# hydradarpa/kalman-hydra

Hardware: AMD Instinct MI355X
Metric: frames/sec (Brox flow + EKF update) at 1024^2 (higher is better)
Workload: dtype f32 (flow, renders) / f64 (EKF sums and state)

## Files before the change

include/hydra_mi.h:

```cpp
#ifndef HYDRA_MI_H
#define HYDRA_MI_H

#include <stdint.h>

#ifdef __cplusplus
extern "C" {
#endif

#define HM_OK 0
#define HM_ERR_ARG (-1)
#define HM_ERR_HIP (-2)
#define HM_ERR_STATE (-3)
#define HM_ERR_NUMERIC (-4)

const char *hm_last_error(void);
const char *hm_version(void);
int hm_device_count(void);

int hm_dev_alloc(int device, uint64_t bytes, void **out);
int hm_dev_free(int device, void *ptr);
int hm_dev_upload(int device, void *dst, const void *src, uint64_t bytes);
int hm_dev_download(int device, void *dst, const void *src, uint64_t bytes);
int hm_copy_stream_create(int device, void **stream_out);
int hm_copy_stream_destroy(int device, void *stream);
// ... 75 lines not shown
int hm_update_step(hm_ctx_t h, const double *X, double deltaX, int masked, double *step, double *Hzc,
                   double err[4]);
int hm_update_cov(hm_ctx_t h, int which, double *W_out);
int hm_update_run(hm_ctx_t h, const double *W_prior, double *X, double deltaX, int masked, int max_iter,
                  double reltol, int info[4], double *errs, double *Hzc, double *gains, double *W_out);
int hm_cov_fetch(hm_ctx_t h, double *W_out);
int hm_ms_newton(int n_vertices, int n_bars, const int32_t *bars, const double *l0, double kappa, double M,
                 double dt, int maxiter, double tol, double *X, int *newton_iterations);
int hm_ms_worker_create(void **worker);
int hm_ms_worker_destroy(void *worker);
int hm_ms_newton_start(void *worker, int n_vertices, int n_bars, const int32_t *bars, const double *l0, double kappa,
                       double M, double dt, int maxiter, double tol, const double *X);
int hm_ms_newton_finish(void *worker, double *X, int *newton_iterations);
int hm_ms_worker_attach(void *worker, hm_ctx_t ctx);
int hm_newton_dev_start(hm_ctx_t h, int N, int n_bars, const int32_t *bars, const double *l0, double kappa, double M,
                        double dt, int maxiter, double tol, const double *X);
int hm_newton_dev_finish(hm_ctx_t h, double *X, int *newton_iterations);
int hm_update_arm_newton(hm_ctx_t h, void *worker, int n_bars, const int32_t *bars, const double *l0, double kappa,
                         double M, double dt, int maxiter, double tol);
int hm_update_arm_cov(hm_ctx_t h, double eps_F);
int hm_predict_take(hm_ctx_t h, const double *X, int n_bars, const int32_t *bars, const double *l0, double kappa,
                    double a, double s, double eps_F);
int hm_cov_predict(hm_ctx_t h, const double *W_in, int n_bars, const int32_t *bars, const double *blocks,
                   double a, double s, double eps_F, double *W_out);
int hm_ms_predict(hm_ctx_t h, int n_bars, const int32_t *bars, const double *l0, double kappa, double M, double dt,
                  int maxiter, double tol, double eps_F, double *X, int *newton_iterations, int prefactor);
int hm_update_last_error(hm_ctx_t h, const double *X, double err[4]);
int hm_chain_project(hm_ctx_t h);
int hm_prepare_mask(hm_ctx_t h, const uint8_t *d_y_m);
int hm_update_arm_mask(hm_ctx_t h, const uint8_t *d_y_m);
int hm_update_tail(hm_ctx_t h, double *Hzc, double *gains);
int hm_chain_states(hm_ctx_t h, double *predicted, double *projected, int *newton_iterations, int *moved);
int hm_ctx_tune(hm_ctx_t h, const char *key, int value);
int hm_ctx_sync(hm_ctx_t h);
void *hm_ctx_stream(hm_ctx_t h);

typedef struct hm_smooth *hm_smooth_t;
int hm_smooth_create(hm_ctx_t ctx, int capacity, int n_bars, const int32_t *bars, const double *l0, double kappa,
                     double a, double s, double eps_F, hm_smooth_t *out);
int hm_smooth_destroy(hm_smooth_t sm);
int hm_smooth_record(hm_smooth_t sm, const double *X);
int hm_smooth_run(hm_smooth_t sm, int want_cov, double *xs, double *var);
int hm_smooth_count(hm_smooth_t sm, int *frames, int *capacity);
int hm_smooth_fetch(hm_smooth_t sm, int k, double *P_out, double *x_out, double *m_out);
int hm_smooth_prior(hm_smooth_t sm, int k, double *Pp_out);
int hm_op_smooth_gemm(int device, int which, int n, const double *A, const double *B, const double *C, double *out);

int hm_view(hm_ctx_t h, const double *X, int which, const int32_t *palette, uint8_t *bgr);
int hm_view_dev(hm_ctx_t h, const double *X, int which, const int32_t *palette, void *d_bgr, void *stream);
int hm_view_forces(hm_ctx_t h, const double *X, const double *orig, const double *pred, const double *tv,
                   const double *fv, const double *mv, uint8_t *bgr);

int hm_view_set_cells(hm_ctx_t h, int n_layers, const int32_t *labels, const uint16_t *weights, int L, const uint8_t *colours);
int hm_view_cells(hm_ctx_t h, const double *X, const uint8_t *frame, const uint8_t *levels, int flags,
                  int P, const double *points, const uint8_t *point_colours, int point_radius, uint8_t *bgr);
int hm_view_cells_dev(hm_ctx_t h, const double *X, const void *d_frame, const uint8_t *levels, int flags,
                      int P, const double *points, const uint8_t *point_colours, int point_radius, void *d_bgr, void *stream);

int hm_body_map(hm_ctx_t h, int32_t *tri_of_pixel, uint32_t *tri_counts);
int hm_body_set_labels(hm_ctx_t h, const int32_t *labels, int L, uint32_t *counts);
int hm_body_warp(hm_ctx_t h, const double *X, const uint8_t *frame, uint8_t *out, uint64_t *tri_sums, uint64_t *label_sums);
int hm_body_warp_dev(hm_ctx_t h, const double *X, const void *d_frame, void *d_out, int out_channels,
                     void *d_tri_sums, void *d_label_sums, void *stream);
int hm_body_fence(hm_ctx_t h, void *stream);

int hm_body_stats_begin(hm_ctx_t h);
// ... 42 lines not shown
```

kalman-hydra_amd/_lib.py:

```python
import ctypes
import os

import numpy as np

_HERE = os.path.dirname(os.path.abspath(__file__))
SO_PATH = os.environ.get("HYDRA_MI_SO") or os.path.join(_HERE, "libhydra_mi.so")

c_f32p = ctypes.POINTER(ctypes.c_float)
c_f64p = ctypes.POINTER(ctypes.c_double)
c_u8p = ctypes.POINTER(ctypes.c_uint8)
c_i32p = ctypes.POINTER(ctypes.c_int32)
c_vp = ctypes.c_void_p

SIGNATURES = {
    "hm_last_error": (ctypes.c_char_p, []),
    "hm_version": (ctypes.c_char_p, []),
    "hm_device_count": (ctypes.c_int, []),
    "hm_dev_alloc": (ctypes.c_int, [ctypes.c_int, ctypes.c_uint64, ctypes.POINTER(c_vp)]),
    "hm_dev_free": (ctypes.c_int, [ctypes.c_int, c_vp]),
    "hm_dev_upload": (ctypes.c_int, [ctypes.c_int, c_vp, c_vp, ctypes.c_uint64]),
    "hm_dev_download": (ctypes.c_int, [ctypes.c_int, c_vp, c_vp, ctypes.c_uint64]),
    "hm_copy_stream_create": (ctypes.c_int, [ctypes.c_int, ctypes.POINTER(c_vp)]),
    "hm_copy_stream_destroy": (ctypes.c_int, [ctypes.c_int, c_vp]),
    "hm_copy_stream_sync": (ctypes.c_int, [ctypes.c_int, c_vp]),
# ... 50 lines not shown
    "hm_update_run": (ctypes.c_int, [c_vp, c_vp, c_vp, ctypes.c_double, ctypes.c_int, ctypes.c_int, ctypes.c_double,
                                     ctypes.POINTER(ctypes.c_int), c_vp, c_vp, c_vp, c_vp]),
    "hm_update_last_error": (ctypes.c_int, [c_vp, c_vp, c_f64p]),
    "hm_cov_fetch": (ctypes.c_int, [c_vp, c_vp]),
    "hm_project_mask": (ctypes.c_int, [c_vp, c_vp, c_vp, c_vp]),
    "hm_cov_predict": (ctypes.c_int, [c_vp, c_vp, ctypes.c_int, c_vp, c_vp, ctypes.c_double, ctypes.c_double,
                                      ctypes.c_double, c_vp]),
    "hm_ms_newton": (ctypes.c_int, [ctypes.c_int, ctypes.c_int, c_vp, c_vp, ctypes.c_double, ctypes.c_double,
                                    ctypes.c_double, ctypes.c_int, ctypes.c_double, c_vp, ctypes.POINTER(ctypes.c_int)]),
    "hm_ms_worker_create": (ctypes.c_int, [ctypes.POINTER(c_vp)]),
    "hm_ms_worker_destroy": (ctypes.c_int, [c_vp]),
    "hm_ms_newton_start": (ctypes.c_int, [c_vp, ctypes.c_int, ctypes.c_int, c_vp, c_vp, ctypes.c_double, ctypes.c_double,
                                          ctypes.c_double, ctypes.c_int, ctypes.c_double, c_vp]),
    "hm_ms_newton_finish": (ctypes.c_int, [c_vp, c_vp, ctypes.POINTER(ctypes.c_int)]),
    "hm_ms_worker_attach": (ctypes.c_int, [c_vp, c_vp]),
    "hm_newton_dev_start": (ctypes.c_int, [c_vp, ctypes.c_int, ctypes.c_int, c_vp, c_vp, ctypes.c_double, ctypes.c_double,
                                           ctypes.c_double, ctypes.c_int, ctypes.c_double, c_vp]),
    "hm_newton_dev_finish": (ctypes.c_int, [c_vp, c_vp, ctypes.POINTER(ctypes.c_int)]),
    "hm_prune_mask": (ctypes.c_int, [c_vp, c_vp, c_vp]),
    "hm_chain_project": (ctypes.c_int, [c_vp]),
    "hm_prepare_mask": (ctypes.c_int, [c_vp, c_vp]),
    "hm_update_arm_mask": (ctypes.c_int, [c_vp, c_vp]),
    "hm_update_tail": (ctypes.c_int, [c_vp, c_vp, c_vp]),
    "hm_chain_states": (ctypes.c_int, [c_vp, c_vp, c_vp, ctypes.POINTER(ctypes.c_int), ctypes.POINTER(ctypes.c_int)]),
    "hm_update_arm_newton": (ctypes.c_int, [c_vp, c_vp, ctypes.c_int, c_vp, c_vp, ctypes.c_double, ctypes.c_double,
                                            ctypes.c_double, ctypes.c_int, ctypes.c_double]),
    "hm_update_arm_cov": (ctypes.c_int, [c_vp, ctypes.c_double]),
    "hm_predict_take": (ctypes.c_int, [c_vp, c_vp, ctypes.c_int, c_vp, c_vp, ctypes.c_double, ctypes.c_double,
                                       ctypes.c_double, ctypes.c_double]),
    "hm_ms_predict": (ctypes.c_int, [c_vp, ctypes.c_int, c_vp, c_vp, ctypes.c_double, ctypes.c_double, ctypes.c_double,
                                     ctypes.c_int, ctypes.c_double, ctypes.c_double, c_vp, ctypes.POINTER(ctypes.c_int),
                                     ctypes.c_int]),
    "hm_ctx_tune": (ctypes.c_int, [c_vp, ctypes.c_char_p, ctypes.c_int]),
    "hm_ctx_sync": (ctypes.c_int, [c_vp]),
    "hm_ctx_stream": (c_vp, [c_vp]),
    "hm_smooth_create": (ctypes.c_int, [c_vp, ctypes.c_int, ctypes.c_int, c_vp, c_vp, ctypes.c_double, ctypes.c_double,
                                        ctypes.c_double, ctypes.c_double, ctypes.POINTER(c_vp)]),
    "hm_smooth_destroy": (ctypes.c_int, [c_vp]),
    "hm_smooth_record": (ctypes.c_int, [c_vp, c_vp]),
    "hm_smooth_run": (ctypes.c_int, [c_vp, ctypes.c_int, c_vp, c_vp]),
    "hm_smooth_count": (ctypes.c_int, [c_vp, c_i32p, c_i32p]),
    "hm_smooth_fetch": (ctypes.c_int, [c_vp, ctypes.c_int, c_vp, c_vp, c_vp]),
    "hm_smooth_prior": (ctypes.c_int, [c_vp, ctypes.c_int, c_vp]),
    "hm_op_smooth_gemm": (ctypes.c_int, [ctypes.c_int, ctypes.c_int, ctypes.c_int, c_vp, c_vp, c_vp, c_vp]),
    "hm_view": (ctypes.c_int, [c_vp, c_vp, ctypes.c_int, c_vp, c_vp]),
    "hm_view_dev": (ctypes.c_int, [c_vp, c_vp, ctypes.c_int, c_vp, c_vp, c_vp]),
    "hm_view_forces": (ctypes.c_int, [c_vp, c_vp, c_vp, c_vp, c_vp, c_vp, c_vp, c_vp]),
    "hm_view_set_cells": (ctypes.c_int, [c_vp, ctypes.c_int, c_vp, c_vp, ctypes.c_int, c_vp]),
    "hm_view_cells": (ctypes.c_int, [c_vp, c_vp, c_vp, c_vp, ctypes.c_int, ctypes.c_int, c_vp, c_vp, ctypes.c_int, c_vp]),
    "hm_view_cells_dev": (ctypes.c_int, [c_vp, c_vp, c_vp, c_vp, ctypes.c_int, ctypes.c_int, c_vp, c_vp, ctypes.c_int, c_vp,
                                         c_vp]),
    "hm_body_map": (ctypes.c_int, [c_vp, c_vp, c_vp]),
    "hm_body_set_labels": (ctypes.c_int, [c_vp, c_vp, ctypes.c_int, c_vp]),
    "hm_body_warp": (ctypes.c_int, [c_vp, c_vp, c_vp, c_vp, c_vp, c_vp]),
    "hm_body_warp_dev": (ctypes.c_int, [c_vp, c_vp, c_vp, c_vp, ctypes.c_int, c_vp, c_vp, c_vp]),
    "hm_body_fence": (ctypes.c_int, [c_vp, c_vp]),
    "hm_body_stats_begin": (ctypes.c_int, [c_vp]),
    "hm_body_stats_end": (ctypes.c_int, [c_vp]),
    "hm_body_stats_count": (ctypes.c_int, [c_vp, c_vp]),
    "hm_body_stats_fetch": (ctypes.c_int, [c_vp, c_vp, c_vp, c_vp, c_vp]),
    "hm_body_stats_images": (ctypes.c_int, [c_vp, c_vp, c_vp, c_vp, c_vp]),
    "hm_body_stats_peaks": (ctypes.c_int, [c_vp, ctypes.c_int, ctypes.c_int, ctypes.c_double, ctypes.c_int, c_vp, c_vp,
                                           c_vp]),
    "hm_body_rec_begin": (ctypes.c_int, [c_vp, ctypes.c_uint64]),
    "hm_body_rec_end": (ctypes.c_int, [c_vp]),
    "hm_body_rec_count": (ctypes.c_int, [c_vp, c_vp]),
# ... 121 lines not shown
```

kalman-hydra_amd/csrc/ctx.h:

```cpp
#pragma once
#include "hm_common.h"
#include "hm_types.h"
#include <chrono>
#include <condition_variable>
#include <functional>
#include <mutex>
#include <thread>
#include <vector>

struct Helper {
    std::thread th;
    std::mutex m;
    std::condition_variable cv;
    std::function<int()> job;
    bool posted = false, busy = false, quit = false;
    int rc = HM_OK;
    char err[512] = "";
    void run()
    {
        std::unique_lock<std::mutex> lk(m);
        for (;;) {
            cv.wait(lk, [&] { return quit || posted; });
            if (quit) return;
            posted = false;
// ... 124 lines not shown
    float *d_yfx, *d_yfy, *d_yfxm, *d_yfym;
    bool obs_owned = true;
    const uint8_t *o_yim, *o_ym;
    const float *o_yfx, *o_yfy;
    bool have_tex, have_obs, have_ref;
    Targets ref, P, Q;
    TriSetup *d_setup, *d_cfgs;
    int4 *d_ubox;
    int *d_tlist = nullptr, *d_tcount = nullptr;
    unsigned *d_tmask = nullptr;
    double *d_X, *d_out, *d_partial;
    uint8_t *d_im8, *d_m8;
    std::vector<double> X0;
    double *d_HTH;
    double *d_H, *d_Hz, *d_Hzc, *d_invW0, *d_Af[2], *d_T[2], *d_step, *d_Wtmp, *d_X0, *d_Xn, *d_Wprior, *d_gain, *d_Awork, *d_Lt[2];
    std::vector<double> upd_X0;
    int upd_last = -1, upd_prev = -1;
    double *d_Wres;
    double *pin;
    size_t pin_n;
    int *pin_scratch;
    std::vector<double> resv, tailv;
    int result_delay = 0;
    bool tail_pending = false;
    bool tail_valid = false;
    long long tail_ticket = 0;
    hipStream_t tail_stream = nullptr;
    Armed armed;
    std::vector<int> sp_h_off, sp_h_bar, sp_h_other;
    std::vector<double> sp_h_blk;
    std::vector<int32_t> sp_bars_cached;
    std::vector<int> tri;
    DPool pool;
    int *d_area;
    int *d_sp_off, *d_sp_bar, *d_sp_other;
    double *d_sp_blk;
    bool upd_open;
    bool prefactored;
    std::vector<double> h_partial;
    int red_blocks = 512;
    double *d_tpart = nullptr;
    std::vector<double> h_tpart;
    int ntiles = 0;
    int render_rows = RI_H;
    bool last_err_valid = false;
    double last_err[4] = {0, 0, 0, 0};
    std::vector<double> last_err_X;
    long long run_ticket;
    int vsplit = 5, esplit;
    std::vector<int32_t> pn_bars;
    std::vector<double> pn_l0;
    double pn_par[4] = {0, 0, 0, 0};
    int pn_maxiter = 0;
    double pq_eps_F = 0.0;
    bool pq_valid = false;
    std::vector<double> pq_X, pq_l0;
    std::vector<int32_t> pq_bars;
    double pq_par[4] = {0, 0, 0, 0};
    hipStream_t stream3 = nullptr;
    int *d_n4nbr = nullptr, *d_n4nbb = nullptr, *d_n4bars = nullptr;
    double *d_n4l0 = nullptr;
    int n4deg = 0;
    std::vector<int32_t> n4_bars;
    std::vector<double> n4_l0;
    double *pin_n4 = nullptr;
    double *d_n4X = nullptr;
// ... 127 lines not shown
```

kalman-hydra_amd/csrc/dense_kernels.h:

```cpp
#pragma once
#include <hip/hip_runtime.h>
#include "ekf_kernels.h"
#include "host_block.h"

#define DNB 32
#define TTT_PF 3

__device__ __forceinline__ double d_rsqrt(double d)
{
    const double r = __builtin_amdgcn_rsq(d);
    const double e = fma(-(d * r), r, 1.0);
#ifdef HM_RSQRT_ORDER2
    return fma(r * 0.5, e, r);
#else
    return fma(r, fma(e, 0.375, 0.5) * e, r);
#endif
}

__device__ __forceinline__ double d_readlane(double v, int lane)
{
    const int lo = __builtin_amdgcn_readlane(__double2loint(v), lane);
    const int hi = __builtin_amdgcn_readlane(__double2hiint(v), lane);
    return __hiloint2double(hi, lo);
}
// ... 460 lines not shown
            const int i = e / DNB, j = e % DNB;
            W[i][j] = (i < nd && j < nd) ? invW0[(size_t)i * n + j] + H[(size_t)i * n + j] : (i == j ? 1.0 : 0.0);
        }
        __syncthreads();
        if (threadIdx.x < 64) chol32_tinv_wave(W, Lt, threadIdx.x);
        return;
    }
    if (row >= n) {
        if (row != rhs_row)
            for (int j = threadIdx.x; j < n; j += 256) A[(size_t)row * n + j] = 0.0;
        return;
    }
    double acc = 0.0;
    for (int j = threadIdx.x; j < n; j += 256) {
        const double h = H[(size_t)row * n + j];
        A[(size_t)row * n + j] = invW0[(size_t)row * n + j] + h;
        acc += h * (X0[j] + -1.0 * X[j]);
    }
    for (int o = 32; o > 0; o >>= 1) acc += __shfl_down(acc, o, 64);
    if ((threadIdx.x & 63) == 0) s[threadIdx.x >> 6] = acc;
    __syncthreads();
    if (threadIdx.x == 0) A[(size_t)rhs_row * n + row] = Hz[row] - (((s[0] + s[1]) + s[2]) + s[3]);
}

#define RES_HEAD 10

__global__ __launch_bounds__(256) void k_iter_result(const double *__restrict__ step, int n, const double *__restrict__ partial,
                                                     int ntiles, const int *__restrict__ overflow,
                                                     const unsigned *__restrict__ flow_ctl, double *__restrict__ res, double ticket,
                                                     int delay_us)
{
    __shared__ double sp[RI_GROUPS * RI_NV];
    __shared__ double sums[RI_NV];
    const int t = threadIdx.x;
    const unsigned long long stamp = hb_stamp((long long)ticket);
    d_tile_partial_sums(partial, ntiles, sp, sums);
    __syncthreads();
    double v = 0.0;
    int slot = -1;
    if (t < 4) { slot = t; v = sums[t]; }
    else if (t == 4) { slot = 4; v = (double)*overflow; }
    else if (t == 5) { slot = 5; v = ticket; }
    else if (t == 6) { slot = 6; v = 0.0; }
    else if (t == 7) { slot = 7; v = (double)flow_ctl[1]; }
    else if (t == 8) { slot = 8; v = sums[4]; }
    else if (t == 9) { slot = 9; v = sums[5]; }
    if (delay_us > 0) {
        if (t == 9) { hb_put(res, n + 9, v, stamp); hb_flush(); }
        hb_delay(delay_us);
    }
    for (int i = t; i < n; i += 256) hb_put(res, i, step[i], stamp);
    if (slot >= 0) hb_put(res, n + slot, v, stamp);
    hb_flush();
}

__global__ __launch_bounds__(256) void k_gains(const double *__restrict__ W, const double *__restrict__ Hzc, int n,
                                               double *__restrict__ out)
{
    __shared__ double sm[3][4];
    const int row = blockIdx.x;
    double a0 = 0.0, a1 = 0.0, a2 = 0.0;
    for (int j = threadIdx.x; j < n; j += 256) {
        const double w = W[(size_t)row * n + j];
        const double *c = Hzc + (size_t)4 * j;
        a0 += w * c[0];
        a1 += w * (c[1] + c[2]);
        a2 += w * c[3];
    }
    for (int o = 32; o > 0; o >>= 1) {
        a0 += __shfl_down(a0, o, 64);
        a1 += __shfl_down(a1, o, 64);
        a2 += __shfl_down(a2, o, 64);
    }
    if ((threadIdx.x & 63) == 0) {
        sm[0][threadIdx.x >> 6] = a0;
        sm[1][threadIdx.x >> 6] = a1;
        sm[2][threadIdx.x >> 6] = a2;
    }
    __syncthreads();
    if (threadIdx.x < 3) {
        const double *q = sm[threadIdx.x];
        out[(size_t)threadIdx.x * n + row] = ((q[0] + q[1]) + q[2]) + q[3];
    }
}

__global__ __launch_bounds__(1024) void k_tail_result(const double *__restrict__ Hzc, const double *__restrict__ gain, int n,
// ... 67 lines not shown
```

kalman-hydra_amd/csrc/ekf.hip:

```cpp
#include "ctx.h"
#include "ekf_kernels.h"
#include "dense_kernels.h"
#include "chol_flow_kernels.h"
#include "project_kernels.h"
#include "predict_kernels.h"
#include "smooth_kernels.h"
#include <algorithm>
#include <atomic>
#include <chrono>
#include <cmath>
#include <cstring>
#include <set>
#include <thread>
#include <utility>
#include <vector>


static int hb_wait(hipStream_t st, const double *blk, size_t first, size_t n, unsigned long long stamp, double *out, const char *who)
{
    const volatile unsigned long long *canary = (const volatile unsigned long long *)blk + 2 * (first + n - 1);
    const auto t_start = std::chrono::steady_clock::now();
    const auto t_yield = t_start + std::chrono::microseconds(700), t_give_up = t_start + std::chrono::milliseconds(20);
    bool polite = false;
    for (int spin = 0;; spin++) {
// ... 1 lines not shown
        if (polite) std::this_thread::yield();
        else __builtin_ia32_pause();
        if ((spin & 255) == 255) {
            const auto now = std::chrono::steady_clock::now();
            if (now > t_give_up) break;
            polite = now > t_yield;
        }
    }
    HM_HIP(hipStreamSynchronize(st));
    if (hb_take(blk, first, n, stamp, out)) return HM_OK;
    hm_set_error("%s: a result block of the device is not whole although its stream has completed (stamp %016llx)", who, stamp);
    return HM_ERR_HIP;
}

static hipError_t pool_alloc(hm_ctx *h, long long cap)
{
    const size_t pc = (size_t)cap;
    h->pool.cap = 0;
    hipError_t e = h->own.grow(&h->pool.live, (pc / 64 + 1) * sizeof(int));
    for (short2 **q : {&h->pool.xi, &h->pool.yi})
        if (e == hipSuccess) e = h->own.grow(q, pc * sizeof(short2));
    for (float **q : {&h->pool.xfx, &h->pool.xfy, &h->pool.yfx, &h->pool.yfy, &h->pool.vxfx, &h->pool.vyfy})
        if (e == hipSuccess) e = h->own.grow(q, pc * sizeof(float));
    if (e == hipSuccess) h->pool.cap = cap;
    return e;
}
static int pool_grow(hm_ctx *h, const char *who)
{
    std::vector<int> area(h->N);
    HM_HIP(hipMemcpyAsync(area.data(), h->d_area, (size_t)h->N * sizeof(int), hipMemcpyDeviceToHost, h->stream));
    HM_HIP(hipStreamSynchronize(h->stream));
    long long total = 0;
    for (int a : area) total += a;
    if (total <= h->pool.cap) { hm_set_error("%s: the difference-image pool reported an overflow it does not have", who); return HM_ERR_STATE; }
    const long long want = total + total / 4;
    if (want > ((long long)1 << 32)) {
        hm_set_error("%s: the star regions need %lld pixels of difference images, more than the pool may hold", who, total);
        return HM_ERR_STATE;
    }
    if (getenv("HYDRA_MI_TRACE")) fprintf(stderr, "[hydra_mi] %s: difference-image pool %lld -> %lld pixels\n", who, h->pool.cap, want);
    const hipError_t e = pool_alloc(h, want);
    if (e != hipSuccess) {
        hm_set_error("%s: cannot grow the difference-image pool to %lld pixels: %s", who, want, hipGetErrorString(e));
        return HM_ERR_HIP;
    }
    return HM_OK;
}

static int ctx_free(hm_ctx *h)
{
    if (!h) return HM_OK;
    (void)ctx_join(h);
    if (h->helper_used) h->helper.stop();
    (void)hipSetDevice(h->device);
    h->own.drain();
    h->own.release();
    delete h;
    return HM_OK;
}


extern "C" int hm_ctx_create(int device, int W, int H, int N, int T, const int32_t *tri, const float *uv, double eps_Z,
                             double eps_J, double eps_M, hm_ctx_t *out)
{
    HM_ARG(out != nullptr, "hm_ctx_create: out is NULL");
    *out = nullptr;
// ... 86 lines not shown
        dev(&h->d_im8, n);
        dev(&h->d_m8, n);
        const size_t n4 = (size_t)4 * N, nn = n4 * n4 * sizeof(double);
        dev(&h->d_H, nn);
        dev(&h->d_HTH, nn);
        if (e == hipSuccess) e = hipMemsetAsync(h->d_HTH, 0, nn, h->stream);
        dev(&h->d_invW0, nn);
        const size_t nn_aug = (size_t)(hm_cdiv((int)n4, DNB) * DNB + DNB) * n4 * sizeof(double);
        dev(&h->d_Af[0], nn_aug);
        dev(&h->d_Af[1], nn_aug);
        dev(&h->d_Awork, nn_aug);
        const size_t ld_bytes = (size_t)hm_cdiv((int)n4, DNB) * DNB * DNB * sizeof(double);
        dev(&h->d_T[0], nn);
        dev(&h->d_T[1], nn);
        dev(&h->d_step, n4 * sizeof(double));
        dev(&h->d_Lt[0], ld_bytes);
        dev(&h->d_Lt[1], ld_bytes);
        dev(&h->d_Wtmp, nn);
        dev(&h->d_flowP, 3 * ld_bytes);
        dev(&h->d_flowctl, 4 * sizeof(unsigned));
        if (e == hipSuccess) e = hipMemsetAsync(h->d_flowctl, 0, 4 * sizeof(unsigned), h->stream);
        dev(&h->d_Hz, n4 * sizeof(double));
        dev(&h->d_Hzc, n4 * 4 * sizeof(double));
        dev(&h->d_Wprior, nn);
        dev(&h->d_gain, n4 * 3 * sizeof(double));
        h->pin_n = 2 * (n4 + RES_HEAD + n4 * 4 + n4 * 3) + 2;
        if (e == hipSuccess) e = h->own.host_alloc(&h->pin, h->pin_n * sizeof(double), hipHostMallocCoherent);
        if (e == hipSuccess) memset(h->pin, 0, h->pin_n * sizeof(double));
        h->pin_scratch = (int *)(h->pin + h->pin_n - 2);
        h->resv.assign(n4 + RES_HEAD, 0.0);
        h->tailv.assign(n4 * 7, 0.0);
        dev(&h->d_X0, n4 * sizeof(double));
        dev(&h->pool.hdr, (size_t)4 * N * sizeof(int));
        dev(&h->pool.overflow, sizeof(int));
        dev(&h->d_area, (size_t)N * sizeof(int));
        h->pool.area = h->d_area;
        if (e == hipSuccess) e = pool_alloc(h, (long long)8 * W * H);
        dev(&h->d_Xn, n4 * sizeof(double));
        for (Targets *t : {&h->ref, &h->P, &h->Q})
            if (e == hipSuccess) e = alloc_targets(h->own, *t, n);
    }
    if (e != hipSuccess) {
        hm_set_error("hm_ctx_create: device allocation failed: %s", hipGetErrorString(e));
        step(HM_ERR_HIP);
    }
    if (rc != HM_OK) {
        ctx_free(h);
        return rc;
    }
    h->h_partial.resize((size_t)h->red_blocks * 4);
    h->h_tpart.resize((size_t)h->ntiles * RI_NV);
    *out = h;
    return HM_OK;
}

extern "C" int hm_ctx_destroy(hm_ctx_t h) { return ctx_free(h); }

void ekf_queue_setup_all(hipStream_t st, const Mesh &m, const double *d_X, TriSetup *d_setup)
{
    hipLaunchKernelGGL(k_setup_all, dim3(hm_cdiv(m.T, 64)), dim3(64), 0, st, m, d_X, d_setup);
}
void ekf_queue_render(hipStream_t st, const Mesh &m, const double *d_X, const TriSetup *d_setup, const Targets &out,
                      const int *d_labels, int *d_ids)
{
    const dim3 grid(hm_cdiv(m.W, EKF_TILE), hm_cdiv(m.H, EKF_TILE)), block(EKF_TILE, EKF_TILE);
    if (d_ids) hipLaunchKernelGGL((k_render<1>), grid, block, 0, st, m, d_X, d_setup, out, d_labels, d_ids);
    else hipLaunchKernelGGL((k_render<0>), grid, block, 0, st, m, d_X, d_setup, out, (const int *)nullptr, (int *)nullptr);
}

#ifdef HM_STAMP
extern "C" int hm_debug_stamps(void *dev_ptr)
{
    long long *p = (long long *)dev_ptr;
    HM_HIP(hipMemcpyToSymbol(HIP_SYMBOL(g_stamp), &p, sizeof p));
    return HM_OK;
}
#endif

extern "C" int hm_ctx_tune(hm_ctx_t h, const char *key, int value)
{
    HM_ARG(h != nullptr && key != nullptr, "hm_ctx_tune: NULL argument");
    HM_JOIN(h);
    if (!strcmp(key, "measure_split")) {
        HM_ARG(value >= 1 && value <= MEAS_VSPLIT_MAX, "hm_ctx_tune: measure_split must be in 1..%d", MEAS_VSPLIT_MAX);
        h->vsplit = value;
    } else if (!strcmp(key, "chol_flow")) {
        HM_ARG(value == 0 || value == 1, "hm_ctx_tune: chol_flow must be 0 (one launch per block step) or 1 (one persistent launch)");
        h->chol_flow = value;
    } else if (!strcmp(key, "chol_flow_wgs")) {
        HM_ARG(value >= 2 && value <= 2048, "hm_ctx_tune: chol_flow_wgs must be in 2..2048 (the chain workgroup and at least one task workgroup)");
        h->flow_wgs = value;
    } else if (!strcmp(key, "render_rows")) {
        HM_ARG(value == 8 || value == 16, "hm_ctx_tune: render_rows must be 8 or 16");
        h->render_rows = value;
    } else if (!strcmp(key, "chol_flow_stall")) {
        HM_ARG(value >= 0 && value <= 100000, "hm_ctx_tune: chol_flow_stall must be in 0..100000");
        h->flow_stall = value;
    } else if (!strcmp(key, "result_delay")) {
        HM_ARG(value >= 0 && value <= 5000, "hm_ctx_tune: result_delay must be in 0..5000 (microseconds)");
        h->result_delay = value;
    } else if (!strcmp(key, "tail_async")) {
        HM_ARG(value == 0 || value == 1, "hm_ctx_tune: tail_async must be 0 or 1");
        h->tail_async = value;
    } else if (!strcmp(key, "tail_split")) {
        HM_ARG(value == 0 || value == 1, "hm_ctx_tune: tail_split must be 0 or 1");
        h->tail_split = value;
    } else if (!strcmp(key, "newton_fail")) {
        HM_ARG(value == 0 || value == 1, "hm_ctx_tune: newton_fail must be 0 or 1");
        h->newton_fail = value;
    } else if (!strcmp(key, "speculate")) {
        HM_ARG(value == 0 || value == 1, "hm_ctx_tune: speculate must be 0 or 1");
        h->speculate = value;
    } else if (!strcmp(key, "edge_split")) {
        HM_ARG(value >= 1 && value <= MEAS_VSPLIT_MAX, "hm_ctx_tune: edge_split must be in 1..%d", MEAS_VSPLIT_MAX);
        h->esplit = value;
    } else if (!strcmp(key, "body_stats_cap")) {
        HM_ARG(value >= 1 && value <= BODY_STATS_CAP, "hm_ctx_tune: body_stats_cap must be in 1..%d", BODY_STATS_CAP);
        h->body.stats_cap = value;
    } else if (!strcmp(key, "body_rec_chunk")) {
        HM_ARG(value >= 0, "hm_ctx_tune: body_rec_chunk must be >= 0 (0: the default size)");
        h->rec.chunk = value;
    } else if (!strcmp(key, "rec_tp_frames")) {
        HM_ARG(value >= 1 && value <= REC_TP_MAX, "hm_ctx_tune: rec_tp_frames must be in 1..%d", REC_TP_MAX);
        h->rec.tp_frames = value;
    } else if (!strcmp(key, "rec_bl_frames")) {
        HM_ARG(value >= 1 && value <= REC_BL_MAX, "hm_ctx_tune: rec_bl_frames must be in 1..%d", REC_BL_MAX);
        h->rec.bl_frames = value;
    } else {
        hm_set_error("hm_ctx_tune: unknown key '%s'", key);
        return HM_ERR_ARG;
    }
    return HM_OK;
}
extern "C" void *hm_ctx_stream(hm_ctx_t h)
{
    (void)ctx_join(h);
    return h ? (void *)h->stream : nullptr;
}
extern "C" int hm_ctx_sync(hm_ctx_t h)
{
    HM_ARG(h != nullptr, "hm_ctx_sync: NULL handle");
    HM_JOIN(h);
    HM_HIP(hipSetDevice(h->device));
    HM_HIP(hipStreamSynchronize(h->stream));
    return HM_OK;
// ... 380 lines not shown
    HM_HIP(hipStreamSynchronize(h->stream));
    for (int l = 0; l < n_labels; l++) {
        const double *s = h->h_lout.data() + 5 * l;
        const double c[4] = {s[0] / h->eps_Z, s[1] / h->eps_J, s[2] / h->eps_J, s[3] / h->eps_M};
        hsum[l] = ((c[0] + c[1]) + c[2]) + c[3];
        nz[l] = s[4];
        if (hcomp) for (int k = 0; k < 4; k++) hcomp[4 * l + k] = c[k];
    }
    return HM_OK;
}

extern "C" int hm_error(hm_ctx_t h, const double *X, int masked, double err[4], float *fx, float *fy)
{
    HM_ARG(h && X && err, "hm_error: NULL argument");
    HM_JOIN(h);
    NEED_TEX(h, "hm_error");
    NEED_OBS(h, "hm_error");
    HM_HIP(hipSetDevice(h->device));
    HM_HIP(hipMemcpyAsync(h->d_X, X, (size_t)4 * h->N * sizeof(double), hipMemcpyHostToDevice, h->stream));
    int rc = render_iter(h, h->d_X, h->P, true, masked, false, 2.0);
    if (rc) return rc;
    const int n = h->W * h->H;
    if (fx) HM_HIP(hipMemcpyAsync(fx, h->P.fx, (size_t)n * sizeof(float), hipMemcpyDeviceToHost, h->stream));
    if (fy) HM_HIP(hipMemcpyAsync(fy, h->P.fy, (size_t)n * sizeof(float), hipMemcpyDeviceToHost, h->stream));
    HM_HIP(hipMemcpyAsync(h->h_tpart.data(), h->d_tpart, (size_t)render_strips(h) * RI_NV * sizeof(double), hipMemcpyDeviceToHost, h->stream));
    HM_HIP(stream_wait(h->stream));
    double s6[RI_NV];
    hm_tile_partial_sums(h->h_tpart.data(), render_strips(h), s6);
    for (int k = 0; k < 4; k++) err[k] = s6[k];
    return HM_OK;
}

static int measure_dev(hm_ctx *h, const double *dX, bool ref_ready, double deltaX, int masked, bool regions_ready = false,
                       bool scatter = true)
{
    if (!ref_ready) {
        int rc = render_iter(h, dX, h->ref, false, masked, !regions_ready, deltaX);
        if (rc) return rc;
        regions_ready = true;
    }
    MeasureArgs a;
    measure_args(h, dX, deltaX, masked, a);
    if (!regions_ready) hipLaunchKernelGGL(k_star_regions, dim3(h->N), dim3(REGION_NT), 0, h->stream, a, h->d_area);
    hipLaunchKernelGGL(k_measure_vertex, dim3(h->N, h->vsplit), dim3(MEAS_NT), 0, h->stream, a,
                       (const TriSetup *)h->d_cfgs, (const int4 *)h->d_ubox, (const unsigned *)h->d_tmask);
    if (h->E > 0) hipLaunchKernelGGL(k_measure_edge, dim3(h->E, h->esplit), dim3(MEAS_NT), 0, h->stream, a);
    if (scatter) {
        ScatterArgs s = {h->d_out, h->d_edges, h->N, h->E, h->vsplit, h->esplit, h->eps_Z, h->eps_J, h->eps_M, deltaX, h->d_HTH, h->d_Hz, h->d_Hzc};
        hipLaunchKernelGGL(k_hth_scatter, dim3(hm_cdiv(h->njobs, 4)), dim3(256), 0, h->stream, s);
    }
    HM_HIP(hipGetLastError());
    return HM_OK;
}

static void measure_args(hm_ctx *h, const double *dX, double deltaX, int masked, MeasureArgs &a)
{
    a.m = Mesh{h->W, h->H, h->N, h->T, h->d_tri, h->d_uv, h->d_tex};
    a.topo = StarTopo{h->d_star_off, h->d_star_tri, h->d_edges, h->E};
    a.ref = h->ref;
    a.obs = obs_of(h, masked);
    a.X = dX;
    a.delta = deltaX;
    a.out = h->d_out;
    a.pool = h->pool;
    a.vsplit = h->vsplit;
    a.esplit = h->esplit;
    a.iZ = 1.0 / h->eps_Z; a.iJ = 1.0 / h->eps_J; a.iM = 1.0 / h->eps_M;
    a.cfgs = h->d_cfgs;
    a.ubox = h->d_ubox;
    a.tmask = h->d_tmask;
    a.tlist = h->d_tlist;
    a.tcount = h->d_tcount;
    a.tmask_stride = TMASK_STRIDE;
}

static int measure_on_device(hm_ctx *h, const double *X, double deltaX, int masked, bool scatter = true)
{
    HM_HIP(hipMemcpyAsync(h->d_X, X, (size_t)4 * h->N * sizeof(double), hipMemcpyHostToDevice, h->stream));
// ... 416 lines not shown
    const auto dbg_a = std::chrono::steady_clock::now();
    auto dbg_ms = [&]() { return std::chrono::duration<double, std::milli>(std::chrono::steady_clock::now() - dbg_a).count(); };
    double dbg_stage[8] = {0, 0, 0, 0, 0, 0, 0, 0};
    int rc = update_begin(h, W_prior, chained ? nullptr : X);
    if (rc) return rc;
    dbg_stage[0] = dbg_ms();
    const int N = h->N, n4 = 4 * N;
    std::vector<double> X0, Xcur, Xold;
    if (!chained) { X0.assign(X, X + n4); Xcur = X0; Xold = X0; }
    auto chain_collect = [&]() -> int {
        int r = hb_wait(h->stream3, h->pin_n4 + n4, 0, (size_t)n4 + 2, hb_stamp(h->n4_ticket), h->n4v.data(), "hm_update_run (state prediction)");
        h->n4_pending = false;
        if (r) return r;
        r = hb_wait(h->stream3, h->pin_pm + n4, 0, (size_t)n4 + 1, hb_stamp(h->pm_ticket), h->pmv.data(), "hm_update_run (projectmask)");
        if (r) return r;
        h->chain_pred.assign(h->n4v.begin(), h->n4v.begin() + n4);
        h->chain_proj.assign(h->pmv.begin(), h->pmv.begin() + n4);
        h->chain_its = (int)h->n4v[n4];
        h->chain_moved = (int)h->pmv[n4];
        if (h->n4v[n4 + 1] != 0.0) return 2;
        X0 = h->chain_proj; Xcur = X0; Xold = X0;
        h->upd_X0 = X0;
        h->X0 = X0;
        return HM_OK;
    };
    bool collected = !chained;
    if (!chained) HM_HIP(hipMemcpyAsync(h->d_X, h->d_X0, (size_t)n4 * sizeof(double), hipMemcpyDeviceToDevice, h->stream));
    double *const pin_res = h->pin, *const pin_tail = h->pin + 2 * ((size_t)n4 + RES_HEAD);
    const double *const res = h->resv.data();
    int niter = 0, accepted = 0;
    bool reverted = false, conv = false, ref_ready = false, regions_ahead = false, grown = false;
    double eold = 0.0;
    bool spec = false;
    auto unspec = [&]() {
        if (spec) { std::swap(h->ref, h->P); std::swap(h->d_X, h->d_Xn); spec = false; }
    };
    for (int it = 0; it < max_iter; it++) {
        if (!spec) {
            rc = measure_dev(h, h->d_X, ref_ready, deltaX, masked, regions_ahead, false);
            if (rc) return rc;
        }
        spec = false;
        if (next_mask && it == 0) {
            HM_HIP(h->own.event(&h->ev_m0));
            HM_HIP(hipEventRecord(h->ev_m0, h->stream));
        }
        if (collected) h->X0 = Xcur;
        h->have_ref = true;
        const int slot = h->upd_last == 0 ? 1 : 0;
        rc = ctx_join(h);
        if (rc) return rc;
        double *rhs_row = solve_step(h, slot, deltaX);
        regions_ahead = it + 1 < max_iter;
        rc = render_iter(h, h->d_Xn, h->P, true, masked, regions_ahead, deltaX);
        if (rc) return rc;
        hipLaunchKernelGGL(k_iter_result, dim3(1), dim3(256), 0, h->stream, rhs_row, n4, h->d_tpart,
                           render_strips(h), h->pool.overflow, (const unsigned *)h->d_flowctl, pin_res, (double)(++h->run_ticket),
                           h->result_delay);
        HM_HIP(hipGetLastError());
        if (h->speculate && regions_ahead) {
            std::swap(h->ref, h->P);
            std::swap(h->d_X, h->d_Xn);
            spec = true;
            rc = measure_dev(h, h->d_X, true, deltaX, masked, true, false);
            if (rc) { unspec(); return rc; }
        }
        const auto dbg_t0 = std::chrono::steady_clock::now();
        if (next_mask && it == 0) {
            rc = ensure_stream2(h);
            if (rc == HM_OK) { HM_HIP(hipStreamWaitEvent(h->stream2, h->ev_m0, 0)); rc = prepare_mask(h, next_mask); }
            if (rc) { unspec(); return rc; }
            next_mask = nullptr;
        }
        if (!collected) {
            rc = chain_collect();
            if (rc) { unspec(); (void)hipStreamSynchronize(h->stream); return rc; }
            collected = true;
        }
        rc = hb_wait(h->stream, pin_res, 0, (size_t)n4 + RES_HEAD, hb_stamp(h->run_ticket), h->resv.data(), "hm_update_run");
        if (rc) { unspec(); return rc; }
        if (getenv("HYDRA_MI_TRACE")) {
            const double ms = std::chrono::duration<double, std::milli>(std::chrono::steady_clock::now() - dbg_t0).count();
            if (ms > 1.5) fprintf(stderr, "[hydra_mi] hm_update_run: iteration %d waited %.2f ms for its result\n", it, ms);
        }
        if (res[n4 + 4] != 0.0) {
            unspec();
            if (grown) { hm_set_error("hm_update_run: the star regions do not fit the difference-image pool"); return HM_ERR_STATE; }
            if (regions_ahead) {
                MeasureArgs a;
                measure_args(h, h->d_X, deltaX, masked, a);
                hipLaunchKernelGGL(k_star_regions, dim3(h->N), dim3(REGION_NT), 0, h->stream, a, h->d_area);
                HM_HIP(hipGetLastError());
            }
            HM_HIP(hipStreamSynchronize(h->stream));
            rc = pool_grow(h, "hm_update_run");
            if (rc) return rc;
            grown = true;
            regions_ahead = false;
            HM_HIP(hipMemsetAsync(h->d_flowctl, 0, 4 * sizeof(unsigned), h->stream));
            it--;
            continue;
        }
        grown = false;
        h->upd_prev = h->upd_last;
        h->upd_last = slot;
        niter++;
        if (res[n4 + 7] != 0.0) {
            unspec();
            hm_set_error("hm_update_run: the factorisation launch gave up waiting for a block (chol_flow time-out)");
            return HM_ERR_HIP;
        }
        bool finite = true;
        for (int i = 0; i < n4; i++) finite = finite && std::isfinite(res[i]);
        if (!finite) {
            unspec();
            hm_set_error("hm_update_run: the update system inv(W) + HTH is not positive definite "
                         "(non-finite state, covariance or observation?)");
            return HM_ERR_NUMERIC;
        }
        for (int i = 0; i < n4; i++) Xcur[i] = X0[i] + res[i];
        if (errs) for (int k = 0; k < 4; k++) errs[4 * it + k] = res[n4 + k];
        bool flipped = false;
        for (int t = 0; t < h->T && !flipped; t++) {
            const int a = h->tri[3 * t], b = h->tri[3 * t + 1], c = h->tri[3 * t + 2];
            const double ax = Xcur[2 * b] - Xcur[2 * a], ay = Xcur[2 * b + 1] - Xcur[2 * a + 1];
            const double bx = Xcur[2 * c] - Xcur[2 * a], by = Xcur[2 * c + 1] - Xcur[2 * a + 1];
            flipped = ax * by - ay * bx < 0.0;
        }
// ... 794 lines not shown
```

kalman-hydra_amd/csrc/ekf_kernels.h:

```cpp
#pragma once
#include <hip/hip_runtime.h>
#include <stdint.h>
#include "hm_types.h"

__global__ void k_setup_all(Mesh m, const double *__restrict__ X, TriSetup *__restrict__ out)
{
    int t = blockIdx.x * blockDim.x + threadIdx.x;
    if (t >= m.T) return;
    int v0 = m.tri[3 * t], v1 = m.tri[3 * t + 1], v2 = m.tri[3 * t + 2];
    TriSetup s;
    d_tri_setup(s, v0, v1, v2, d_snap(X[2 * v0]), d_snap(X[2 * v0 + 1]), d_snap(X[2 * v1]), d_snap(X[2 * v1 + 1]),
                d_snap(X[2 * v2]), d_snap(X[2 * v2 + 1]), m.W, m.H);
    d_tri_attr(s, m.uv, X, m.N);
    out[t] = s;
}

template <int MODE>
__global__ __launch_bounds__(EKF_TILE *EKF_TILE) void k_render(Mesh m, const double *__restrict__ X,
                                                                const TriSetup *__restrict__ setup, Targets out,
                                                                const int *__restrict__ labels, int *__restrict__ ids)
{
    __shared__ unsigned s_mask[EKF_MAX_TRI / 32];
    const int tid = threadIdx.y * EKF_TILE + threadIdx.x;
    const int words = (m.T + 31) / 32;
    for (int i = tid; i < words; i += EKF_TILE * EKF_TILE) s_mask[i] = 0;
    __syncthreads();
    const int c0 = blockIdx.x * EKF_TILE, r0 = blockIdx.y * EKF_TILE;
    for (int t = tid; t < m.T; t += EKF_TILE * EKF_TILE) {
        const TriSetup &s = setup[t];
        if (s.cmin <= s.cmax && s.cmax >= c0 && s.cmin < c0 + EKF_TILE && s.rmax >= r0 && s.rmin < r0 + EKF_TILE)
            atomicOr(&s_mask[t >> 5], 1u << (t & 31));
    }
    __syncthreads();
    const int c = c0 + threadIdx.x, r = r0 + threadIdx.y;
    if (c >= m.W || r >= m.H) return;
    int acc = 0, cnt = 0, sg = 0, sb = 0;
// ... 457 lines not shown
        if (word != 0) a.tlist[(size_t)v * a.tmask_stride + before + __popcll(bal & ((1ull << lane) - 1ull))] = t;
        for (int w = 0; w < NW; w++) listed += sh.wsum[w];
    }
    if (threadIdx.x == 0) a.tcount[v] = listed;
}

__global__ __launch_bounds__(REGION_NT) void k_star_regions(MeasureArgs a, int *__restrict__ area)
{
    __shared__ RegionShared sh;
    d_star_regions<REGION_NT>(a, area, blockIdx.x, sh);
}

template <int NT>
__device__ inline void d_region_sums(const int *__restrict__ area, int N, int v, int w, long long &bv, long long &bw,
                                     long long &tot, long long *s )
{
    long long a = 0, b = 0, c = 0;
    for (int i = threadIdx.x; i < N; i += NT) {
        const long long x = area[i];
        c += x;
        if (i < v) a += x;
        if (i < w) b += x;
    }
    for (int o = 32; o > 0; o >>= 1) {
        a += __shfl_down(a, o, 64); b += __shfl_down(b, o, 64); c += __shfl_down(c, o, 64);
    }
    const int lane = threadIdx.x & 63, wv = threadIdx.x >> 6;
    if (lane == 0) { s[wv * 3] = a; s[wv * 3 + 1] = b; s[wv * 3 + 2] = c; }
    __syncthreads();
    bv = 0; bw = 0; tot = 0;
    for (int k = 0; k < NT / 64; k++) { bv += s[k * 3]; bw += s[k * 3 + 1]; tot += s[k * 3 + 2]; }
}

#ifndef MEAS_OCC
#define MEAS_OCC 4
#endif
__global__ __launch_bounds__(MEAS_NT, MEAS_OCC) void k_measure_vertex(MeasureArgs a, const TriSetup *__restrict__ cfgs,
                                                                const int4 *__restrict__ ubox, const unsigned *__restrict__ tmask)
{
    __shared__ double s_red[(MEAS_NT / 64) * MEAS_OUT];
    __shared__ double s_k255[511];
    const double *k255 = s_k255 + 255;
    d_fill_k255(s_k255, MEAS_NT);
    const Mesh &m = a.m;
    const int N = m.N, W = m.W;
    const int v = blockIdx.x, job = v;
    const double *X = a.X;
    const double d = a.delta;
    const int nsv = a.topo.star_off[v + 1] - a.topo.star_off[v];
    const TriSetup *__restrict__ s_cfg[MEAS_NCFG];
#pragma unroll
    for (int c = 0; c < MEAS_NCFG; c++) s_cfg[c] = cfgs + ((size_t)v * MEAS_NCFG + c) * (EKF_MAX_STAR + 1);
    __syncthreads();
    const int c0 = a.pool.hdr[4 * v], r0 = a.pool.hdr[4 * v + 1], rw = a.pool.hdr[4 * v + 2], rh = a.pool.hdr[4 * v + 3];
    __shared__ long long s_sum[(MEAS_NT / 64) * 3];
    long long base, unused, total;
    d_region_sums<MEAS_NT>(a.pool.area, N, v, 0, base, unused, total, s_sum);
    const bool park = total <= a.pool.cap;
    if (v == 0 && blockIdx.y == 0 && threadIdx.x == 0) *a.pool.overflow = park ? 0 : 1;
    double acc[A_NV];
#pragma unroll
    for (int k = 0; k < A_NV; k++) acc[k] = 0.0;
    const int wave = __builtin_amdgcn_readfirstlane(threadIdx.x >> 6);
    const int lx = threadIdx.x & 7, ly = (threadIdx.x & 63) >> 3;
    const int ntx = (rw + 7) >> 3, ntiles = ntx * ((rh + 7) >> 3);
    const int nwaves = (MEAS_NT / 64) * gridDim.y;
    const int listed = a.tcount[v];
    const int nwalk = listed >= 0 ? listed : ntiles;
    for (int j = blockIdx.y * (MEAS_NT / 64) + wave; j < nwalk; j += nwaves) {
        const int tile = listed >= 0 ? a.tlist[(size_t)v * a.tmask_stride + j] : j;
        const int tr0 = r0 + 8 * (tile / ntx), tc0 = c0 + 8 * (tile % ntx);
        const int r = tr0 + ly, c = tc0 + lx;
        unsigned mask = 0;
        if (listed >= 0) {
            mask = tmask[(size_t)v * a.tmask_stride + tile];
        } else {
            for (int k = 0; k < nsv; k++) {
                const int4 b = ubox[(size_t)v * UBOX_STRIDE + k];
                if (!((b.y < tc0) | (b.x > tc0 + 7) | (b.w < tr0) | (b.z > tr0 + 7))) mask |= 1u << k;
// ... 339 lines not shown
            e[5] += (double)gfy * (double)gfy;
        }
    }
    HM_STAMP_AT(3);
    if (!r.with_err) return;
    d_block_reduce<RI_NV, 256>(e, sh.t.red, r.partial + RI_NV * (size_t)tile);
    HM_STAMP_AT(4);
}

__device__ __forceinline__ void d_tile_partial_sums(const double *__restrict__ partial, int ntiles, double *sp, double *out)
{
    const int t = threadIdx.x;
    if (t < RI_GROUPS) {
        double s[RI_NV];
#pragma unroll
        for (int k = 0; k < RI_NV; k++) s[k] = 0.0;
#pragma unroll 4
        for (int i = t; i < ntiles; i += RI_GROUPS) {
            const double2 *q = (const double2 *)(partial + RI_NV * (size_t)i);
#pragma unroll
            for (int k = 0; k < RI_NV / 2; k++) { const double2 v = q[k]; s[2 * k] += v.x; s[2 * k + 1] += v.y; }
        }
#pragma unroll
        for (int k = 0; k < RI_NV; k++) sp[RI_NV * t + k] = s[k];
    }
    __syncthreads();
    if (t < RI_NV) {
        double s = 0.0;
        for (int g = 0; g < RI_GROUPS; g++) s += sp[RI_NV * g + t];
        out[t] = s;
    }
}

struct ScatterArgs {
    const double *out;
    const int *edges;
    int N, E, vsplit, esplit;
    double eZ, eJ, eM, d;
    double *H, *Hz, *Hzc;
};

__device__ __forceinline__ void d_put(double *H, int n4, int p, int q, double val, double d)
{
    const double v = val / d / d;
    H[(size_t)p * n4 + q] = v;
    H[(size_t)q * n4 + p] = v;
}

__global__ __launch_bounds__(256) void k_hth_scatter(ScatterArgs a)
{
    __shared__ double so[4][MEAS_OUT];
    const int wv = threadIdx.x >> 6, lane = threadIdx.x & 63;
    const int job = blockIdx.x * 4 + wv;
    const int N = a.N, n4 = 4 * N;
    const bool on = job < N + a.E;
    if (on && lane < MEAS_OUT) {
        const double *src = a.out + (size_t)job * MEAS_VSPLIT_MAX * MEAS_OUT;
        const int parts = job < N ? a.vsplit : a.esplit;
        double v = src[lane];
        for (int q = 1; q < parts; q++) v += src[q * MEAS_OUT + lane];
        so[wv][lane] = v;
    }
    __syncthreads();
    if (!on) return;
    const double *o = so[wv];
    const double eZ = a.eZ, eJ = a.eJ, eM = a.eM, d = a.d;
// ... 54 lines not shown
```

Baseline: 333.8.

## Fold iteration-result kernel into speculative measure launch as an extra block

Result: no change. 336.6 (median of 3 runs) (+0.9%).

```diff
diff --git a/include/hydra_mi.h b/include/hydra_mi.h
--- a/include/hydra_mi.h
+++ b/include/hydra_mi.h
@@ -131,6 +131,7 @@
 int hm_update_tail(hm_ctx_t h, double *Hzc, double *gains);
 int hm_chain_states(hm_ctx_t h, double *predicted, double *projected, int *newton_iterations, int *moved);
 int hm_ctx_tune(hm_ctx_t h, const char *key, int value);
+int hm_pool_stats(hm_ctx_t h, long long out[4]);
 int hm_ctx_sync(hm_ctx_t h);
 void *hm_ctx_stream(hm_ctx_t h);
 
diff --git a/kalman-hydra_amd/_lib.py b/kalman-hydra_amd/_lib.py
--- a/kalman-hydra_amd/_lib.py
+++ b/kalman-hydra_amd/_lib.py
@@ -106,6 +106,7 @@
                                      ctypes.c_int, ctypes.c_double, ctypes.c_double, c_vp, ctypes.POINTER(ctypes.c_int),
                                      ctypes.c_int]),
     "hm_ctx_tune": (ctypes.c_int, [c_vp, ctypes.c_char_p, ctypes.c_int]),
+    "hm_pool_stats": (ctypes.c_int, [c_vp, c_vp]),
     "hm_ctx_sync": (ctypes.c_int, [c_vp]),
     "hm_ctx_stream": (c_vp, [c_vp]),
     "hm_smooth_create": (ctypes.c_int, [c_vp, ctypes.c_int, ctypes.c_int, c_vp, c_vp, ctypes.c_double, ctypes.c_double,
diff --git a/kalman-hydra_amd/csrc/ctx.h b/kalman-hydra_amd/csrc/ctx.h
--- a/kalman-hydra_amd/csrc/ctx.h
+++ b/kalman-hydra_amd/csrc/ctx.h
@@ -180,6 +180,10 @@
     std::vector<int32_t> sp_bars_cached;
     std::vector<int> tri;
     DPool pool;
+    long long pool_grows = 0, pool_grow_total = 0;
+    int pool_grow_iter = -1;
+    double *d_ridesp = nullptr;
+    int result_rider = 1;
     int *d_area;
     int *d_sp_off, *d_sp_bar, *d_sp_other;
     double *d_sp_blk;
diff --git a/kalman-hydra_amd/csrc/dense_kernels.h b/kalman-hydra_amd/csrc/dense_kernels.h
--- a/kalman-hydra_amd/csrc/dense_kernels.h
+++ b/kalman-hydra_amd/csrc/dense_kernels.h
@@ -516,26 +516,7 @@
 {
     __shared__ double sp[RI_GROUPS * RI_NV];
     __shared__ double sums[RI_NV];
-    const int t = threadIdx.x;
-    const unsigned long long stamp = hb_stamp((long long)ticket);
-    d_tile_partial_sums(partial, ntiles, sp, sums);
-    __syncthreads();
-    double v = 0.0;
-    int slot = -1;
-    if (t < 4) { slot = t; v = sums[t]; }
-    else if (t == 4) { slot = 4; v = (double)*overflow; }
-    else if (t == 5) { slot = 5; v = ticket; }
-    else if (t == 6) { slot = 6; v = 0.0; }
-    else if (t == 7) { slot = 7; v = (double)flow_ctl[1]; }
-    else if (t == 8) { slot = 8; v = sums[4]; }
-    else if (t == 9) { slot = 9; v = sums[5]; }
-    if (delay_us > 0) {
-        if (t == 9) { hb_put(res, n + 9, v, stamp); hb_flush(); }
-        hb_delay(delay_us);
-    }
-    for (int i = t; i < n; i += 256) hb_put(res, i, step[i], stamp);
-    if (slot >= 0) hb_put(res, n + slot, v, stamp);
-    hb_flush();
+    d_iter_result(step, n, partial, ntiles, overflow, flow_ctl, res, ticket, delay_us, sp, sums);
 }
 
 __global__ __launch_bounds__(256) void k_gains(const double *__restrict__ W, const double *__restrict__ Hzc, int n,
diff --git a/kalman-hydra_amd/csrc/ekf.hip b/kalman-hydra_amd/csrc/ekf.hip
--- a/kalman-hydra_amd/csrc/ekf.hip
+++ b/kalman-hydra_amd/csrc/ekf.hip
@@ -57,6 +57,8 @@
     HM_HIP(hipStreamSynchronize(h->stream));
     long long total = 0;
     for (int a : area) total += a;
+    h->pool_grows++;
+    h->pool_grow_total = total;
     if (total <= h->pool.cap) { hm_set_error("%s: the difference-image pool reported an overflow it does not have", who); return HM_ERR_STATE; }
     const long long want = total + total / 4;
     if (want > ((long long)1 << 32)) {
@@ -209,7 +211,8 @@
         h->tailv.assign(n4 * 7, 0.0);
         dev(&h->d_X0, n4 * sizeof(double));
         dev(&h->pool.hdr, (size_t)4 * N * sizeof(int));
-        dev(&h->pool.overflow, sizeof(int));
+        dev(&h->pool.overflow, 2 * sizeof(int));
+        dev(&h->d_ridesp, (size_t)RI_GROUPS * RI_NV * sizeof(double));
         dev(&h->d_area, (size_t)N * sizeof(int));
         h->pool.area = h->d_area;
         if (e == hipSuccess) e = pool_alloc(h, (long long)8 * W * H);
@@ -232,6 +235,14 @@
 }
 
 extern "C" int hm_ctx_destroy(hm_ctx_t h) { return ctx_free(h); }
+
+extern "C" int hm_pool_stats(hm_ctx_t h, long long out[4])
+{
+    HM_ARG(h && out, "hm_pool_stats: NULL argument");
+    HM_JOIN(h);
+    out[0] = h->pool.cap; out[1] = h->pool_grows; out[2] = h->pool_grow_total; out[3] = h->pool_grow_iter;
+    return HM_OK;
+}
 
 void ekf_queue_setup_all(hipStream_t st, const Mesh &m, const double *d_X, TriSetup *d_setup)
 {
@@ -288,6 +299,12 @@
     } else if (!strcmp(key, "speculate")) {
         HM_ARG(value == 0 || value == 1, "hm_ctx_tune: speculate must be 0 or 1");
         h->speculate = value;
+    } else if (!strcmp(key, "result_rider")) {
+        HM_ARG(value == 0 || value == 1, "hm_ctx_tune: result_rider must be 0 or 1");
+        h->result_rider = value;
+    } else if (!strcmp(key, "pool_cap")) {
+        HM_ARG(value >= 1, "hm_ctx_tune: pool_cap must be >= 1 (pixels)");
+        if (value < h->pool.cap) h->pool.cap = value;
     } else if (!strcmp(key, "edge_split")) {
         HM_ARG(value >= 1 && value <= MEAS_VSPLIT_MAX, "hm_ctx_tune: edge_split must be in 1..%d", MEAS_VSPLIT_MAX);
         h->esplit = value;
@@ -734,7 +751,7 @@
 }
 
 static int measure_dev(hm_ctx *h, const double *dX, bool ref_ready, double deltaX, int masked, bool regions_ready = false,
-                       bool scatter = true)
+                       bool scatter = true, int *ovf = nullptr, const IterResult *ride = nullptr)
 {
     if (!ref_ready) {
         int rc = render_iter(h, dX, h->ref, false, masked, !regions_ready, deltaX);
@@ -743,9 +760,10 @@
     }
     MeasureArgs a;
     measure_args(h, dX, deltaX, masked, a);
+    if (ovf) a.pool.overflow = ovf;
     if (!regions_ready) hipLaunchKernelGGL(k_star_regions, dim3(h->N), dim3(REGION_NT), 0, h->stream, a, h->d_area);
-    hipLaunchKernelGGL(k_measure_vertex, dim3(h->N, h->vsplit), dim3(MEAS_NT), 0, h->stream, a,
-                       (const TriSetup *)h->d_cfgs, (const int4 *)h->d_ubox, (const unsigned *)h->d_tmask);
+    hipLaunchKernelGGL(k_measure_vertex, dim3(h->N + (ride ? 1 : 0), h->vsplit), dim3(MEAS_NT), 0, h->stream, a,
+                       (const TriSetup *)h->d_cfgs, (const int4 *)h->d_ubox, (const unsigned *)h->d_tmask, ride ? *ride : IterResult{});
     if (h->E > 0) hipLaunchKernelGGL(k_measure_edge, dim3(h->E, h->esplit), dim3(MEAS_NT), 0, h->stream, a);
     if (scatter) {
         ScatterArgs s = {h->d_out, h->d_edges, h->N, h->E, h->vsplit, h->esplit, h->eps_Z, h->eps_J, h->eps_M, deltaX, h->d_HTH, h->d_Hz, h->d_Hzc};
@@ -1228,12 +1246,13 @@
     bool reverted = false, conv = false, ref_ready = false, regions_ahead = false, grown = false;
     double eold = 0.0;
     bool spec = false;
+    int ow = 0;
     auto unspec = [&]() {
         if (spec) { std::swap(h->ref, h->P); std::swap(h->d_X, h->d_Xn); spec = false; }
     };
     for (int it = 0; it < max_iter; it++) {
         if (!spec) {
-            rc = measure_dev(h, h->d_X, ref_ready, deltaX, masked, regions_ahead, false);
+            rc = measure_dev(h, h->d_X, ref_ready, deltaX, masked, regions_ahead, false, h->pool.overflow + ow);
             if (rc) return rc;
         }
         spec = false;
@@ -1250,15 +1269,23 @@
         regions_ahead = it + 1 < max_iter;
         rc = render_iter(h, h->d_Xn, h->P, true, masked, regions_ahead, deltaX);
         if (rc) return rc;
-        hipLaunchKernelGGL(k_iter_result, dim3(1), dim3(256), 0, h->stream, rhs_row, n4, h->d_tpart,
-                           render_strips(h), h->pool.overflow, (const unsigned *)h->d_flowctl, pin_res, (double)(++h->run_ticket),
-                           h->result_delay);
-        HM_HIP(hipGetLastError());
-        if (h->speculate && regions_ahead) {
+        const bool go_on = h->speculate && regions_ahead;
+        IterResult result = {};
+        result.step = rhs_row; result.n = n4; result.partial = h->d_tpart; result.ntiles = render_strips(h);
+        result.overflow = h->pool.overflow + ow; result.flow_ctl = (const unsigned *)h->d_flowctl;
+        result.res = pin_res; result.sp = h->d_ridesp; result.ticket = (double)(++h->run_ticket); result.delay_us = h->result_delay;
+        const bool ride = go_on && h->result_rider && !grown;
+        if (!ride) {
+            hipLaunchKernelGGL(k_iter_result, dim3(1), dim3(256), 0, h->stream, result.step, result.n, result.partial, result.ntiles,
+                               result.overflow, result.flow_ctl, result.res, result.ticket, result.delay_us);
+            HM_HIP(hipGetLastError());
+        }
+        if (go_on) {
             std::swap(h->ref, h->P);
             std::swap(h->d_X, h->d_Xn);
             spec = true;
-            rc = measure_dev(h, h->d_X, true, deltaX, masked, true, false);
+            ow ^= 1;
+            rc = measure_dev(h, h->d_X, true, deltaX, masked, true, false, h->pool.overflow + ow, ride ? &result : nullptr);
             if (rc) { unspec(); return rc; }
         }
         const auto dbg_t0 = std::chrono::steady_clock::now();
@@ -1290,6 +1317,7 @@
             }
             HM_HIP(hipStreamSynchronize(h->stream));
             rc = pool_grow(h, "hm_update_run");
+            h->pool_grow_iter = it;
             if (rc) return rc;
             grown = true;
             regions_ahead = false;
diff --git a/kalman-hydra_amd/csrc/ekf_kernels.h b/kalman-hydra_amd/csrc/ekf_kernels.h
--- a/kalman-hydra_amd/csrc/ekf_kernels.h
+++ b/kalman-hydra_amd/csrc/ekf_kernels.h
@@ -2,6 +2,7 @@
 #include <hip/hip_runtime.h>
 #include <stdint.h>
 #include "hm_types.h"
+#include "host_block.h"
 
 __global__ void k_setup_all(Mesh m, const double *__restrict__ X, TriSetup *__restrict__ out)
 {
@@ -525,19 +526,43 @@
     for (int k = 0; k < NT / 64; k++) { bv += s[k * 3]; bw += s[k * 3 + 1]; tot += s[k * 3 + 2]; }
 }
 
+struct IterResult {
+    const double *step;
+    const double *partial;
+    const int *overflow;
+    const unsigned *flow_ctl;
+    long long pad0;
+    double *res;
+    double *sp;
+    long long pad1;
+    double ticket;
+    int n, ntiles, delay_us;
+};
+__device__ __forceinline__ void d_iter_result(const double *__restrict__ step, int n, const double *__restrict__ partial, int ntiles,
+                                              const int *__restrict__ overflow, const unsigned *__restrict__ flow_ctl,
+                                              double *__restrict__ res, double ticket, int delay_us, double *sp, double *sums);
+
 #ifndef MEAS_OCC
 #define MEAS_OCC 4
 #endif
 __global__ __launch_bounds__(MEAS_NT, MEAS_OCC) void k_measure_vertex(MeasureArgs a, const TriSetup *__restrict__ cfgs,
-                                                                const int4 *__restrict__ ubox, const unsigned *__restrict__ tmask)
+                                                                const int4 *__restrict__ ubox, const unsigned *__restrict__ tmask,
+                                                                IterResult ride)
 {
     __shared__ double s_red[(MEAS_NT / 64) * MEAS_OUT];
     __shared__ double s_k255[511];
+    const int rider = ride.res != nullptr ? 1 : 0;
+    if (rider && blockIdx.x == 0) {
+        if (blockIdx.y == 0)
+            d_iter_result(ride.step, ride.n, ride.partial, ride.ntiles, ride.overflow, ride.flow_ctl, ride.res, ride.ticket,
+                          ride.delay_us, ride.sp, s_red);
+        return;
+    }
     const double *k255 = s_k255 + 255;
     d_fill_k255(s_k255, MEAS_NT);
     const Mesh &m = a.m;
     const int N = m.N, W = m.W;
-    const int v = blockIdx.x, job = v;
+    const int v = blockIdx.x - rider, job = v;
     const double *X = a.X;
     const double d = a.delta;
     const int nsv = a.topo.star_off[v + 1] - a.topo.star_off[v];
@@ -943,6 +968,34 @@
     }
 }
 
+static_assert(MEAS_NT == 256 && RI_GROUPS == 256 && (MEAS_NT / 64) * MEAS_OUT >= RI_NV,
+              "d_iter_result: 256 threads; the rider keeps its RI_NV totals in k_measure_vertex's s_red");
+__device__ __forceinline__ void d_iter_result(const double *__restrict__ step, int n, const double *__restrict__ partial, int ntiles,
+                                              const int *__restrict__ overflow, const unsigned *__restrict__ flow_ctl,
+                                              double *__restrict__ res, double ticket, int delay_us, double *sp, double *sums)
+{
+    const int t = threadIdx.x;
+    const unsigned long long stamp = hb_stamp((long long)ticket);
+    d_tile_partial_sums(partial, ntiles, sp, sums);
+    __syncthreads();
+    double v = 0.0;
+    int slot = -1;
+    if (t < 4) { slot = t; v = sums[t]; }
+    else if (t == 4) { slot = 4; v = (double)*overflow; }
+    else if (t == 5) { slot = 5; v = ticket; }
+    else if (t == 6) { slot = 6; v = 0.0; }
+    else if (t == 7) { slot = 7; v = (double)flow_ctl[1]; }
+    else if (t == 8) { slot = 8; v = sums[4]; }
+    else if (t == 9) { slot = 9; v = sums[5]; }
+    if (delay_us > 0) {
+        if (t == 9) { hb_put(res, n + 9, v, stamp); hb_flush(); }
+        hb_delay(delay_us);
+    }
+    for (int i = t; i < n; i += 256) hb_put(res, i, step[i], stamp);
+    if (slot >= 0) hb_put(res, n + slot, v, stamp);
+    hb_flush();
+}
+
 struct ScatterArgs {
     const double *out;
     const int *edges;
```
